# tensorlayer/HyperPose

Measured on NVIDIA H100. Metric: frames/sec end-to-end (conv+PAF parse) OpenPose-COCO 368x656, higher is better.
Workload: dtype f16 operands, f32 accumulate (conv); f32/f64 (parse)

## Files before the change

### hyperpose_b200/capi.py

```python
from __future__ import annotations

import ctypes as C
import os
import struct

import numpy as np

PKG = os.path.dirname(os.path.abspath(__file__))
LIB_PATH = os.path.join(PKG, "libhyperpose_b200.so")

N_PARTS, N_PAIRS = 18, 19
HP_OK, HP_ERR_ARG, HP_ERR_CAPACITY, HP_ERR_UNSUPPORTED, HP_ERR_CUDA, HP_ERR_BATCH = 0, -1, -2, -3, -4, -5

PART_DT = np.dtype({"names": ["has_value", "x", "y", "score"], "formats": ["<i4", "<f4", "<f4", "<f4"]})
HUMAN_DT = np.dtype([("parts", PART_DT, (N_PARTS,)), ("score", "<f4")])
PEAK_DT = np.dtype([("part_id", "<i4"), ("x", "<i4"), ("y", "<i4"), ("score", "<f4"), ("id", "<i4")])
CONN_DT = np.dtype([("cid1", "<i4"), ("cid2", "<i4"), ("score", "<f4")])
assert HUMAN_DT.itemsize == 292

EXPORTS = [
    "hp_last_error", "hp_device_count", "hp_version",
    "hp_paf_create", "hp_paf_destroy", "hp_paf_set_conf_thresh", "hp_paf_set_paf_thresh", "hp_paf_set_capacity",
    "hp_paf_process_host", "hp_paf_process_host_batched", "hp_paf_process_device", "hp_paf_fetch",
    "hp_paf_debug_peaks", "hp_paf_debug_connections", "hp_paf_launch_count", "hp_paf_copy_results_device", "hp_paf_debug_timing",
# ... 151 lines not shown
        _bind_engine(L)
        L._engine_bound = True
    check(L.hp_handoff_enable(1 if on else 0))


EXPORTS += [
    "hp_engine_create", "hp_engine_destroy", "hp_engine_info", "hp_engine_infer_u8_host", "hp_engine_infer_u8_device",
    "hp_engine_infer_f32_host", "hp_engine_outputs", "hp_engine_read_outputs_host", "hp_engine_copy_outputs_device", "hp_engine_sync",
    "hp_engine_launch_count", "hp_engine_debug_read_buffer", "hp_engine_debug_write_buffer", "hp_engine_debug_run_ops",
    "hp_pose_run_u8_host", "hp_engine_stage_frame_u8", "hp_engine_infer_staged", "hp_engine_debug_read_frames", "hp_engine_set_output_override", "hp_engine_set_profiling", "hp_engine_get_profile",
    "hp_engine_read_outputs_frames", "hp_engine_head_type", "hp_handoff_enable", "hp_handoff_stats",
    "hp_pose_submit_u8_host", "hp_pose_collect", "hp_pose_stats", "hp_paf_prepare", "hp_paf_state", "hp_paf_copy_results_host_async",
    "hp_paf_grow_capacity", "hp_pool_create", "hp_pool_destroy", "hp_pool_size", "hp_pool_set_capacity", "hp_pool_run_u8_host",
    "hp_pool_set_output_override", "hp_pool_launch_count", "hp_default_device", "hp_handoff_device_of",
    "hp_engine_create_ex", "hp_engine_dtype", "hp_pose_submit_u8_device", "hp_engine_debug_op_kernel",
    "hp_engine_debug_op_epilogue",
    "hp_engine_calibrate_u8", "hp_pack_int8_calibrated",
]


def _bind_engine(L):
    vp, ip = C.c_void_p, C.POINTER(C.c_int)
    L.hp_engine_create.argtypes = [C.POINTER(vp), vp, C.c_size_t, C.c_int, C.c_int, C.c_int, C.c_double, C.c_int, C.c_int]
    L.hp_engine_create_ex.argtypes = [C.POINTER(vp), vp, C.c_size_t, C.c_int, C.c_int, C.c_int, C.c_double, C.c_int, C.c_int, C.c_int]
    L.hp_engine_dtype.argtypes = [vp]
    L.hp_engine_destroy.argtypes = [vp]
    L.hp_engine_destroy.restype = None
    L.hp_engine_info.argtypes = [vp, ip, ip, ip, ip, ip, ip, ip, C.POINTER(C.c_double)]
    L.hp_engine_infer_u8_host.argtypes = [vp, vp, C.c_int]
    L.hp_engine_infer_u8_device.argtypes = [vp, vp, C.c_int, vp]
    L.hp_engine_infer_f32_host.argtypes = [vp, vp, C.c_int]
    L.hp_engine_outputs.argtypes = [vp, C.POINTER(vp), C.POINTER(vp), C.POINTER(vp)]
    L.hp_engine_read_outputs_host.argtypes = [vp, vp, vp, C.c_int]
    L.hp_engine_sync.argtypes = [vp]
    L.hp_engine_copy_outputs_device.argtypes = [vp, vp, vp, C.c_int, vp]
    L.hp_engine_launch_count.argtypes = [vp]
    L.hp_engine_launch_count.restype = C.c_longlong
    L.hp_engine_debug_read_buffer.argtypes = [vp, C.c_int, vp, C.c_int, ip, ip, ip]
    L.hp_engine_debug_write_buffer.argtypes = [vp, C.c_int, vp, C.c_int]
    L.hp_engine_debug_run_ops.argtypes = [vp, C.c_int, C.c_int, C.c_int]
    L.hp_engine_debug_op_kernel.argtypes = [vp, C.c_int, C.c_char_p, C.c_int]
    L.hp_engine_debug_op_epilogue.argtypes = [vp, C.c_int, ip]
    L.hp_engine_calibrate_u8.argtypes = [vp, vp, C.c_int, vp, C.c_int]
    L.hp_pack_int8_calibrated.argtypes = [vp, C.c_size_t]
    L.hp_pose_run_u8_host.argtypes = [vp, vp, vp, C.c_int, vp, C.c_int, ip]
    L.hp_engine_stage_frame_u8.argtypes = [vp, C.c_int, vp, C.c_int, C.c_int, C.c_int]
    L.hp_engine_infer_staged.argtypes = [vp, C.c_int]
    L.hp_engine_debug_read_frames.argtypes = [vp, vp, C.c_int]
    L.hp_engine_set_output_override.argtypes = [vp, vp, vp]
    L.hp_engine_set_profiling.argtypes = [vp, C.c_int]
    L.hp_engine_get_profile.argtypes = [vp, vp, vp, vp, C.c_int, ip, C.POINTER(C.c_longlong)]
    L.hp_engine_read_outputs_frames.argtypes = [vp, C.POINTER(vp), C.POINTER(vp), C.c_int, C.c_int]
    L.hp_engine_head_type.argtypes = [vp]
    L.hp_handoff_enable.argtypes = [C.c_int]
    L.hp_handoff_stats.argtypes = [C.POINTER(C.c_longlong)] * 4
    L.hp_pose_submit_u8_host.argtypes = [vp, vp, vp, C.c_int, ip]
    L.hp_pose_submit_u8_device.argtypes = [vp, vp, vp, C.c_int, ip]
# ... 143 lines not shown
        return out

    def debug_run_ops(self, first: int, last: int, n: int):
        check(lib().hp_engine_debug_run_ops(self._h, first, last, n))

    def debug_op_kernel(self, op: int) -> str:
        buf = C.create_string_buffer(64)
        check(lib().hp_engine_debug_op_kernel(self._h, op, buf, len(buf)))
        return buf.value.decode()

    def debug_op_epilogue(self, op: int) -> str:
        v = C.c_int(0)
        check(lib().hp_engine_debug_op_epilogue(self._h, op, C.byref(v)))
        return "tma" if v.value else "reg"

    def set_output_override(self, d_conf_ptr: int, d_paf_ptr: int):
        check(lib().hp_engine_set_output_override(self._h, d_conf_ptr, d_paf_ptr))

    def set_profiling(self, enable: bool):
        check(lib().hp_engine_set_profiling(self._h, 1 if enable else 0))

    def get_profile(self):
        cap = 1024
        ms = np.zeros(cap, np.float64); ty = np.zeros(cap, np.int32); fl = np.zeros(cap, np.float64)
        n, runs = C.c_int(), C.c_longlong()
        check(lib().hp_engine_get_profile(self._h, ms.ctypes.data, ty.ctypes.data, fl.ctypes.data, cap, C.byref(n), C.byref(runs)))
        return ms[:n.value], ty[:n.value], fl[:n.value], runs.value

    def run_pose(self, parser: "PafParser", frames: np.ndarray, cap: int = 128):
        frames = np.ascontiguousarray(frames, np.uint8)
# ... 242 lines not shown
```

### hyperpose_b200/csrc/conv_wgmma.cuh

```cuda
#pragma once
#include <cuda.h>
#include <cuda_fp16.h>
#include <cuda_runtime.h>
#include <stdint.h>

#include <type_traits>

namespace hpb {

constexpr int CONV_BLOCK_M = 128;
constexpr int CONV_BLOCK_K = 64;
constexpr int TF32_BLOCK_K = 32;
constexpr int CONV_MAX_STAGES = 8;
constexpr int CONV_THREADS = 384;
constexpr int CONV_A_BYTES = CONV_BLOCK_M * 128;
constexpr size_t CONV_SMEM_LIMIT = 227 * 1024;

enum ConvOutMode : int {
    OUT_F16_NHWC = 0,
    OUT_F32_NCHW_SPLIT = 1,
};

struct ConvParams {
    int Nb, H, W;
// ... 9 lines not shown
    int out_mode;
    void* out; void* out2;
    int out_ld, out_ch_off;
    int split;
    const void* res;
    int res_ld, res_ch_off;
    int res_mode;
    const float* post_w; const float* post_b; const float* post_a;
    const uint8_t* frames;
    int in_h, in_w, stem_stride, stem_pad_h, stem_pad_w, flip;
    double factor;
    float mean[3];
    const float* mul;
    float out_inv_scale, res_scale;
    int in_g_stride;
};

template <typename T> struct ConvAcc { using type = float; };
template <> struct ConvAcc<int8_t> { using type = int; };

namespace ptx {

__device__ __forceinline__ uint32_t smem_u32(const void* p) { return (uint32_t)__cvta_generic_to_shared(p); }

__device__ __forceinline__ void mbar_init(uint32_t bar, uint32_t count)
{
    asm volatile("mbarrier.init.shared::cta.b64 [%0], %1;" ::"r"(bar), "r"(count) : "memory");
}
__device__ __forceinline__ void mbar_expect_tx(uint32_t bar, uint32_t bytes)
{
// ... 51 lines not shown
        "cp.async.bulk.tensor.4d.shared::cluster.global.im2col.mbarrier::complete_tx::bytes [%0], [%1, {%3, %4, %5, %6}], [%2], {%7, %8};"
        ::"r"(dst), "l"(m), "r"(bar), "r"(c), "r"(w), "r"(h), "r"(n), "h"((unsigned short)offw), "h"((unsigned short)offh)
        : "memory");
}
__device__ __forceinline__ void tma_store_2d(const CUtensorMap* m, uint32_t src, int c0, int c1)
{
    asm volatile("cp.async.bulk.tensor.2d.global.shared::cta.bulk_group [%0, {%2, %3}], [%1];" ::"l"(m), "r"(src), "r"(c0), "r"(c1) : "memory");
}
__device__ __forceinline__ void tma_load_2d(uint32_t dst, const CUtensorMap* m, uint32_t bar, int c0, int c1)
{
    asm volatile(
        "cp.async.bulk.tensor.2d.shared::cluster.global.mbarrier::complete_tx::bytes [%0], [%1, {%3, %4}], [%2];"
        ::"r"(dst), "l"(m), "r"(bar), "r"(c0), "r"(c1)
        : "memory");
}
__device__ __forceinline__ void pdl_launch_dependents() { asm volatile("griddepcontrol.launch_dependents;" ::: "memory"); }
__device__ __forceinline__ void pdl_wait() { asm volatile("griddepcontrol.wait;" ::: "memory"); }
__device__ __forceinline__ float round_tf32(float x)
{
    uint32_t r;
    asm("cvt.rna.tf32.f32 %0, %1;" : "=r"(r) : "f"(x));
    return __uint_as_float(r);
}

__device__ __forceinline__ uint64_t make_sw128_kmajor_desc(uint32_t smem_addr)
{
    uint64_t d = 0;
    d |= (uint64_t)((smem_addr & 0x3ffffu) >> 4);
    d |= (uint64_t)1 << 16;
    d |= (uint64_t)(1024u >> 4) << 32;
// ... 265 lines not shown
                }
            }
        }
        vals[j] = __float2half_rn(v);
    }
    const uint4* v4 = (const uint4*)vals;
#pragma unroll
    for (int i = 0; i < 8; ++i) o[i ^ oswz] = v4[i];
}

__device__ __forceinline__ int8_t quantize_i8(float y, float inv_s)
{
    return (int8_t)min(max(__float2int_rn(__fmul_rn(y, inv_s)), -127), 127);
}

template <typename T, int BN, bool kRes, int kStemR = 0>
__global__ void __launch_bounds__(CONV_THREADS, 1)
conv_wgmma_kernel(const __grid_constant__ CUtensorMap tmap_a, const __grid_constant__ CUtensorMap tmap_b, const ConvParams p)
{
    constexpr bool kF16 = std::is_same<T, __half>::value;
    constexpr bool kI8 = std::is_same<T, int8_t>::value;
    constexpr int BK = 128 / (int)sizeof(T);
    constexpr int STAGE_BYTES = CONV_A_BYTES + BN * 128;
    extern __shared__ uint8_t smem_raw[];
    ptx::pdl_launch_dependents();
    uint8_t* smem = (uint8_t*)(((uintptr_t)smem_raw + 1023) & ~(uintptr_t)1023);
    uint64_t* full_bar = (uint64_t*)(smem + (size_t)p.num_stages * STAGE_BYTES);
    uint64_t* empty_bar = full_bar + CONV_MAX_STAGES;

    const int wg = threadIdx.x >> 7, warp = threadIdx.x >> 5, lane = threadIdx.x & 31;
    const int n_tiles_g = p.cout_g_pad / BN;
    const int total_tiles = p.m_tiles * p.groups * n_tiles_g;
    const int chunks = p.cin_g / BK;
    const int ksteps = p.R * p.S * chunks;

    if (threadIdx.x == 0) {
        ptx::prefetch_tmap(&tmap_a);
        ptx::prefetch_tmap(&tmap_b);
        for (int i = 0; i < p.num_stages; ++i) {
            ptx::mbar_init(ptx::smem_u32(full_bar + i), kStemR ? 129 : 1);
            ptx::mbar_init(ptx::smem_u32(empty_bar + i), 8);
        }
        ptx::fence_barrier_init();
    }
    __syncthreads();
    ptx::pdl_wait();

    if constexpr (kStemR > 0) {
        if (wg == 0) {
            const int row = threadIdx.x;
            const int total_px = p.Nb * p.H * p.W;
            int stage = 0;
            uint32_t phase = 0;
// ... 48 lines not shown
                            ptx::mbar_expect_tx(fb, (uint32_t)STAGE_BYTES);
                            ptx::tma_load_im2col_4d(ptx::smem_u32(sa), &tmap_a, fb, a_ch0 + c * BK, q0.w - pad_w, q0.h - pad_h, q0.n, s, r);
                            ptx::tma_load_2d(ptx::smem_u32(sa + CONV_A_BYTES), &tmap_b, fb, kcol, b_row);
                            ring.step(p.num_stages);
                        }
            }
        }
        return;
    }

    const int half = wg - 1;
    const int row0 = half * 64 + (warp & 3) * 16 + (lane >> 2);
    const int col0 = 2 * (lane & 3);
    const int total_px = p.Nb * p.H * p.W;
    const uint32_t smem0 = ptx::smem_u32(smem);
    typename ConvAcc<T>::type acc[BN / 2];
    RingPos ring;
    for (int tile = blockIdx.x; tile < total_tiles; tile += gridDim.x) {
        const ConvTile t = decode_tile(p, tile, n_tiles_g);
        int prev = 0;
        for (int ks = 0; ks < ksteps; ++ks) {
            const uint32_t sa = smem0 + (uint32_t)(ring.slot * STAGE_BYTES);
            const uint64_t da = ptx::make_sw128_kmajor_desc(sa + (uint32_t)(half * 64 * 128)), db = ptx::make_sw128_kmajor_desc(sa + CONV_A_BYTES);
            ptx::mbar_wait(ptx::smem_u32(full_bar + ring.slot), ring.phase);
            ptx::fence_acc(acc);
            ptx::wgmma_fence();
#pragma unroll
            for (int k = 0; k < 4; ++k)
                ptx::wgmma<T, BN>(acc, da + (uint64_t)(k * 2), db + (uint64_t)(k * 2), (ks | k) != 0 ? 1u : 0u);
            ptx::wgmma_commit();
            ptx::fence_acc(acc);
            if (ks > 0) {
                ptx::wgmma_wait<1>();
                if (lane == 0) ptx::mbar_arrive(ptx::smem_u32(empty_bar + prev));
            }
            prev = ring.slot;
            ring.step(p.num_stages);
        }
        ptx::wgmma_wait<0>();
        ptx::fence_acc(acc);
        if (lane == 0) ptx::mbar_arrive(ptx::smem_u32(empty_bar + prev));

        const float* bias = p.bias + t.g * p.cout_g_pad + t.n0;
        const float* alpha = p.alpha + t.g * p.cout_g_pad + t.n0;
        const int n_valid = min(BN, p.cout_g - t.n0);
        const int och = p.out_ch_off + t.g * p.cout_g + t.n0;
        const bool pair_ok = ((och | p.out_ld) & 1) == 0;
#pragma unroll
        for (int h = 0; h < 2; ++h) {
            const int px = t.p0 + row0 + 8 * h;
            if (px >= total_px) continue;
            const size_t pix = (size_t)px;
            const PixelPos q = unflatten(p, px);
#pragma unroll
            for (int j = 0; j < BN / 8; ++j) {
                const int c = 8 * j + col0;
                if (c >= n_valid) break;
// ... 72 lines not shown
                    for (int e = 0; e < 2; ++e) {
                        if (e == 1 && !two) break;
                        const int ch = t.n0 + c + e;
                        const float y = e ? a1 : a0;
                        if (ch < p.split) {
                            ((float*)p.out)[(((size_t)q.n * p.split + ch) * p.H + q.h) * p.W + q.w] = y;
                        } else {
                            const int c2 = ch - p.split, n2 = p.cout_g - p.split;
                            ((float*)p.out2)[(((size_t)q.n * n2 + c2) * p.H + q.h) * p.W + q.w] = y;
                        }
                    }
                }
            }
        }
    }
}

constexpr size_t CONV_SMEM_FIXED = 1024  + 2 * CONV_MAX_STAGES * 8;
inline size_t conv_smem_bytes(int BN, int stages) { return CONV_SMEM_FIXED + (size_t)stages * (CONV_A_BYTES + BN * 128); }
inline int conv_pick_stages(int BN)
{
    int s = CONV_MAX_STAGES;
    while (s > 2 && conv_smem_bytes(BN, s) > CONV_SMEM_LIMIT) --s;
    return s;
}

constexpr int HALO_TH = 16, HALO_TW = 8;

constexpr int HALO_WIDE_PRODUCER_REGS = 40, HALO_WIDE_CONSUMER_REGS = 232;


#ifdef HPB_HALO_PHASES
enum { HALO_PH_TOTAL, HALO_PH_A_WAIT, HALO_PH_B_WAIT, HALO_PH_MMA_WAIT, HALO_PH_EPILOGUE, HALO_PH_TURN_WAIT, HALO_PH_STAGE_WAIT, HALO_PH_COUNT };
__device__ unsigned long long g_halo_phases[HALO_PH_COUNT];
#define HALO_PH_MARK(t) const long long t = clock64()
#define HALO_TIMED(i, ...) do { const long long t0_ = clock64(); __VA_ARGS__; ph[i] += clock64() - t0_; } while (0)
#define HALO_PH_ADD(i, t) (ph[i] += clock64() - (t))
#define HALO_PH_PARAM , long long (&ph)[HALO_PH_COUNT]
// ... 37 lines not shown
}
inline int halo_stage_bytes(int BN, HaloItem it) { return halo_shape(it, BN).stage_slots * BN * 128; }

namespace ptx {
__device__ __forceinline__ uint64_t make_sw128_kmajor_desc_at(uint32_t smem_addr, uint32_t sbo)
{
    uint64_t d = 0;
    d |= (uint64_t)((smem_addr & 0x3ffffu) >> 4);
    d |= (uint64_t)1 << 16;
    d |= (uint64_t)((sbo >> 4) & 0x3fffu) << 32;
    d |= (uint64_t)1 << 62;
    return d;
}
template <uint32_t N> __device__ __forceinline__ void setmaxnreg_dec() { asm volatile("setmaxnreg.dec.sync.aligned.u32 %0;" ::"n"(N)); }
template <uint32_t N> __device__ __forceinline__ void setmaxnreg_inc() { asm volatile("setmaxnreg.inc.sync.aligned.u32 %0;" ::"n"(N)); }
__device__ __forceinline__ void stmatrix_x4(uint32_t addr, uint32_t r0, uint32_t r1, uint32_t r2, uint32_t r3)
{
    asm volatile("stmatrix.sync.aligned.m8n8.x4.shared.b16 [%0], {%1, %2, %3, %4};" ::"r"(addr), "r"(r0), "r"(r1), "r"(r2), "r"(r3) : "memory");
}
__device__ __forceinline__ void st_shared_u32(uint32_t addr, uint32_t v) { asm volatile("st.shared.b32 [%0], %1;" ::"r"(addr), "r"(v) : "memory"); }
__device__ __forceinline__ void named_barrier_sync(int id, int threads) { asm volatile("bar.sync %0, %1;" ::"r"(id), "r"(threads) : "memory"); }
__device__ __forceinline__ void tma_store_4d(const CUtensorMap* m, uint32_t src, int c0, int c1, int c2, int c3)
{
    asm volatile("cp.async.bulk.tensor.4d.global.shared::cta.bulk_group [%0, {%2, %3, %4, %5}], [%1];"
                 ::"l"(m), "r"(src), "r"(c0), "r"(c1), "r"(c2), "r"(c3) : "memory");
}
__device__ __forceinline__ void bulk_commit() { asm volatile("cp.async.bulk.commit_group;" ::: "memory"); }
template <int N> __device__ __forceinline__ void bulk_wait_read() { asm volatile("cp.async.bulk.wait_group.read %0;" ::"n"(N) : "memory"); }
template <int N> __device__ __forceinline__ void bulk_wait() { asm volatile("cp.async.bulk.wait_group %0;" ::"n"(N) : "memory"); }
__device__ __forceinline__ uint32_t half2_bits(__half2 h) { return *reinterpret_cast<uint32_t*>(&h); }
}

template <int BN, bool kPool, int kBlocks>
__device__ __forceinline__ void halo_epilogue(const float (&acc)[kBlocks][BN / 2], const HaloParams& p, int n, int y0, int x0, int g, int n0,
                                              int row_base, int warp, int lane)
{
    const int col0 = 2 * (lane & 3);
    const int tx = lane >> 2;
    const float* bias = p.bias + g * p.cout_g_pad + n0;
    const float* alpha = p.alpha + g * p.cout_g_pad + n0;
    const int och = p.out_ch_off + g * p.cout_g + n0;
    const bool pair_ok = ((och | p.out_ld) & 1) == 0;
    if constexpr (kPool) {
#pragma unroll
        for (int m = 0; m < kBlocks; ++m) {
// ... 398 lines not shown
```

### hyperpose_b200/csrc/engine.cu

```cuda
#include <cuda.h>
#include <cuda_fp16.h>
#include <cuda_runtime.h>
#include <math.h>
#include <stdint.h>
#include <stdlib.h>
#include <string.h>

#include <algorithm>
#include <memory>
#include <string>
#include <vector>

#include "../../include/hyperpose_b200.h"
#include "common.h"
#include "conv_wgmma.cuh"
#include "helpers_tf32_int8.cuh"
#include "handoff.h"
#include "pair_math.cuh"
#include "pack_format.h"

namespace {
using namespace hpb;


// ... 480 lines not shown

int make_tmap_act_box(CUtensorMap* m, const __half* base, int N, int H, int W, int C, int ld, int box_w, int box_h, CUtensorMapSwizzle swizzle)
{
    const auto enc = (PFN_encodeTiled)driver_entry_point("cuTensorMapEncodeTiled");
    if (!enc) { set_error("cuTensorMapEncodeTiled entry point not available"); return HP_ERR_CUDA; }
    cuuint64_t dims[4] = { (cuuint64_t)C, (cuuint64_t)W, (cuuint64_t)H, (cuuint64_t)N };
    cuuint64_t strides[3] = { (cuuint64_t)ld * 2, (cuuint64_t)W * ld * 2, (cuuint64_t)H * W * ld * 2 };
    cuuint32_t box[4] = { 64, (cuuint32_t)box_w, (cuuint32_t)box_h, 1 };
    cuuint32_t estr[4] = { 1, 1, 1, 1 };
    CUresult r = enc(m, CU_TENSOR_MAP_DATA_TYPE_FLOAT16, 4, (void*)base, dims, strides, box, estr, CU_TENSOR_MAP_INTERLEAVE_NONE,
                     swizzle, CU_TENSOR_MAP_L2_PROMOTION_L2_256B, CU_TENSOR_MAP_FLOAT_OOB_FILL_NONE);
    if (r != CUDA_SUCCESS) { set_error("cuTensorMapEncodeTiled(box) failed: %d (N=%d H=%d W=%d C=%d ld=%d box %dx%d)", (int)r, N, H, W, C, ld, box_w, box_h); return HP_ERR_CUDA; }
    return HP_OK;
}

int round_up(int a, int b) { return (a + b - 1) / b * b; }

int pick_bn(int cout_g)
{
    if (cout_g <= 16) return 16;
    if (cout_g <= 32) return 32;
    if (cout_g <= 48) return 48;
    if (cout_g <= 64) return 64;
    if (cout_g <= 96) return 96;
    if (cout_g <= 128) return 128;
    int best = 128;
    for (int bn : { 96, 64 })
        if (round_up(cout_g, bn) < round_up(cout_g, best)) best = bn;
    return best;
}
// ... 52 lines not shown

struct EngOp {
    Launch launch = Launch::None;
    PackOp po;
    ConvPlan plan;
    float* d_dw = nullptr;
    CUtensorMap tmap_dw;
    int dwt_wbo = 0, dwt_hb = 0, dwt_tiles_x = 0, dwt_tiles_y = 0, dwt_stages = 0;
    size_t dwt_smem = 0;
};

struct EngOptions {
    enum { HALO_AUTO, HALO_NONE, HALO_ALL } halo = HALO_AUTO;
    bool halo_wide = true;
    bool halo_tma_store = true;
    bool stem3 = true;
    bool pool_fuse = true;
    bool dw1_fuse = true;
    bool dw_pair = true;
    bool dw_tma = true;
    int pifpaf_reserve_sms = 0;
};

inline int same_pad_before(int in, int k, int stride)
{
    const int out = (in + stride - 1) / stride;
    const int total = std::max((out - 1) * stride + k - in, 0);
    return total / 2;
}

// ... 93 lines not shown
    HaloParams& h = op.plan.hp;
    const int BN = op.plan.prm.BN;
    h.tma_store = e->opt.halo_tma_store && halo_tma_store_ok(h, BN);
    h.stage_bytes = h.tma_store ? halo_stage_bytes(BN, item) : 0;
    h.num_stages = conv_halo_pick_stages(h.R, h.S, BN, item, h.tma_store);
    op.plan.smem = conv_halo_smem_bytes(h.R, h.S, BN, h.num_stages, item, h.tma_store);
    op.plan.halo_item = item;
    op.plan.halo_pool = pool;
    op.launch = Launch::Halo;
    if (!h.tma_store) return HP_OK;
    const int oh = pool ? h.H / 2 : h.H, ow = pool ? h.W / 2 : h.W, box = pool ? HALO_TW / 2 : HALO_TW;
    return make_tmap_act_box(&op.plan.tmap_o, h.out, e->max_batch, oh, ow, h.out_ch_off + h.groups * h.cout_g, h.out_ld, box, box,
                             CU_TENSOR_MAP_SWIZZLE_128B);
}

bool halo_wide_faster(int R, long wide_items, int sms)
{
    return R == 7 && wide_items >= sms;
}

bool halo_pp_exists(int R, int BN) { return R == 3 && (BN == 64 || BN == 128); }
bool halo_pp_faster(int chunks, bool pooled, long items, int sms) { return (chunks >= 4 || pooled) && items >= 2L * sms; }

HaloItem pick_halo_item(const hp_engine* e, const EngOp& op, bool pooled)
{
    const HaloParams& h = op.plan.hp;
    const int BN = op.plan.prm.BN, sms = e->num_sms - e->reserve_sms;
    const long tiles = (long)h.Nb * h.tiles_x * h.tiles_y, n_tiles = (long)h.groups * (h.cout_g_pad / BN);
    const bool all = e->opt.halo == EngOptions::HALO_ALL;
    if (!e->opt.halo_wide) return HaloItem::Narrow;
// ... 73 lines not shown
    }
    HP_CUDA_TRY(cudaMalloc(&pl.d_w, w.size() * es));
    HP_CUDA_TRY(cudaMalloc(&pl.d_bias, bias.size() * sizeof(float)));
    HP_CUDA_TRY(cudaMalloc(&pl.d_alpha, alpha.size() * sizeof(float)));
    HP_CUDA_TRY(cudaMemcpy(pl.d_w, tf32 ? (const void*)w.data() : i8 ? (const void*)wq.data() : (const void*)wh.data(), w.size() * es, cudaMemcpyHostToDevice));
    HP_CUDA_TRY(cudaMemcpy(pl.d_bias, bias.data(), bias.size() * sizeof(float), cudaMemcpyHostToDevice));
    HP_CUDA_TRY(cudaMemcpy(pl.d_alpha, alpha.data(), alpha.size() * sizeof(float), cudaMemcpyHostToDevice));

    ConvParams& p = pl.prm;
    memset(&p, 0, sizeof(p));
    p.Nb = e->max_batch; p.H = ib.H; p.W = ib.W;
    p.R = eR; p.S = eS; p.groups = G; p.cin_g = ecin;
    p.cout_g = cout_g; p.cout_g_pad = cout_pad; p.BN = BN;
    p.m_tiles = (int)(((size_t)e->max_batch * p.H * p.W + CONV_BLOCK_M - 1) / CONV_BLOCK_M);
    p.in_ch_off = (int)po.in_ch_off;
    p.num_stages = conv_pick_stages(BN);
    p.bias = pl.d_bias; p.alpha = pl.d_alpha;
    p.out_mode = (int)po.out_mode;
    if (po.out_mode == OUT_F32_NCHW_SPLIT) {
        p.out = e->d_conf; p.out2 = e->d_paf; p.split = (int)po.split;
        if ((int)po.split != (int)e->hdr.conf_channels || cout_g - (int)po.split != (int)e->hdr.paf_channels || G != 1) {
            set_error("engine: output conv must produce conf(%u)+paf(%u) channels", e->hdr.conf_channels, e->hdr.paf_channels);
            return HP_ERR_ARG;
        }
        if (e->hdr.head_type != 0 || ib.H != e->out_h || ib.W != e->out_w) {
            set_error("engine: output conv op %d reads a %dx%d buffer but the outputs are %dx%d conf/paf planes (head_type %u)",
                      (int)(&op - e->ops.data()), ib.H, ib.W, e->out_h, e->out_w, e->hdr.head_type);
            return HP_ERR_ARG;
        }
    } else {
        const EngBuffer& ob = e->bufs[po.out_buf];
// ... 1 lines not shown
        p.out = ob.d; p.out_ld = ob.channels; p.out_ch_off = (int)po.out_ch_off;
        if (i8) p.out_inv_scale = 1.0f / e->act_scale[po.out_buf];
    }
    if (i8) { p.mul = pl.d_mul; p.in_g_stride = cin_g; }
    if (po.res_mode) {
        if (po.out_mode != OUT_F16_NHWC || po.res_buf >= e->bufs.size()) { set_error("engine: bad residual"); return HP_ERR_ARG; }
        const EngBuffer& rb = e->bufs[po.res_buf];
        if (rb.H != ib.H || rb.W != ib.W || (int)po.res_ch_off + G * cout_g > rb.channels || po.res_ch_off % 8 || cout_g % 16) { set_error("engine: residual buffer mismatch"); return HP_ERR_ARG; }
        p.res = rb.d; p.res_ld = rb.channels; p.res_ch_off = (int)po.res_ch_off; p.res_mode = (int)po.res_mode;
        if (i8) p.res_scale = e->act_scale[po.res_buf];
    }
    int rc = make_tmap_act_im2col(&pl.tmap_a, ib.d, e->max_batch, ib.H, ib.W, ib.channels, eR, eS, e->dtype);
    if (rc) return rc;
    rc = make_tmap_wgt(&pl.tmap_b, pl.d_w, G * cout_pad, K, BN, e->dtype);
    if (rc) return rc;
    pl.smem = conv_smem_bytes(BN, p.num_stages);
    pl.flops_per_frame = 2.0 * ib.H * ib.W * (double)G * cout_g * cin_g * R * S;
    op.launch = Launch::Conv;
    if (e->dtype != HP_DTYPE_F16) return HP_OK;
    pl.monotone_act = true;
    for (float a : alpha) if (!(a >= 0.f)) { pl.monotone_act = false; break; }
    const int ty = (ib.H + HALO_TH - 1) / HALO_TH, tx = (ib.W + HALO_TW - 1) / HALO_TW;
    const double waste = (double)ty * HALO_TH * tx * HALO_TW / ((double)ib.H * ib.W) - 1.0;
    const bool shape_ok = !im2col && eR == eS && (eR == 3 || eR == 5 || eR == 7) && !po.res_mode && po.out_mode == OUT_F16_NHWC;
    const bool rounds = (long)p.m_tiles * G * (cout_pad / BN) > e->num_sms - e->reserve_sms;
    const bool faster = (eR == 3 && waste <= 0.06) || (rounds && ecin >= 2 * CONV_BLOCK_K && waste <= 0.25);
    const bool want = e->opt.halo == EngOptions::HALO_AUTO ? faster : e->opt.halo == EngOptions::HALO_ALL;
    if (shape_ok && want) {
        const EngBuffer& ob = e->bufs[po.out_buf];
        HaloParams& h = pl.hp;
        memset(&h, 0, sizeof(h));
// ... 100 lines not shown
        HaloParams h = pl.hp;
        h.Nb = N;
        const int tiles = halo_shape(pl.halo_item, p.BN).tiles;
        const long items = ((long)N * h.tiles_x * h.tiles_y + tiles - 1) / tiles * h.groups * (h.cout_g_pad / p.BN);
        cudaLaunchAttribute at[1];
        const cudaLaunchConfig_t cfg = pdl_config((int)std::min<long>(e->num_sms - e->reserve_sms, items), CONV_THREADS, pl.smem, st, at);
        void* args[] = { (void*)&pl.tmap_x, (void*)&pl.tmap_b, (void*)&pl.tmap_o, (void*)&h };
        HP_CUDA_TRY(cudaLaunchKernelExC(&cfg, halo_kernel(p.BN, pl.halo_item, pl.halo_pool), args));
        return HP_OK;
    }
    p.m_tiles = (int)(((size_t)N * p.H * p.W + CONV_BLOCK_M - 1) / CONV_BLOCK_M);
    const int n_tiles = p.m_tiles * p.groups * (p.cout_g_pad / p.BN);
    const int grid = std::min(e->num_sms - e->reserve_sms, n_tiles);
    cudaLaunchAttribute at[1];
    const cudaLaunchConfig_t cfg = pdl_config(grid, CONV_THREADS, pl.smem, st, at);
    void* args[] = { (void*)&pl.tmap_a, (void*)&pl.tmap_b, (void*)&p };
    HP_CUDA_TRY(cudaLaunchKernelExC(&cfg, conv_kernel(e->dtype, p.res_mode != 0, p.BN, stem_R), args));
    return HP_OK;
}

bool collect_one(hp_engine* e, bool blocking)
{
    if (e->ev_tail >= e->ev_head) return false;
    const size_t n = e->ops.size();
    cudaEvent_t* set = e->ev.data() + (size_t)(e->ev_tail % hp_engine::EV_DEPTH) * (n + 1);
    if (!blocking && cudaEventQuery(set[n]) != cudaSuccess) { cudaGetLastError(); return false; }
    cudaEventSynchronize(set[n]);
    for (size_t i = 0; i < n; ++i) {
        float ms = 0.f;
        if (cudaEventElapsedTime(&ms, set[i], set[i + 1]) == cudaSuccess) e->op_ms_sum[i] += ms;
    }
// ... 321 lines not shown
        }
    }
    HP_CUDA_TRY(cudaSetDevice(device));
    cudaDeviceProp prop;
    HP_CUDA_TRY(cudaGetDeviceProperties(&prop, device));
    if (prop.major != 9) { set_error("hp_engine_create: device is sm_%d%d; this engine is wgmma/TMA code for sm_90a only", prop.major, prop.minor); return HP_ERR_UNSUPPORTED; }

    hp_engine* e = new hp_engine();
    e->device = device; e->dtype = dtype; e->in_h = in_h; e->in_w = in_w; e->max_batch = max_batch;
    e->factor = factor; e->flip_rgb = flip_rgb; e->hdr = hdr; e->num_sms = prop.multiProcessorCount;
    e->act_scale = std::move(act_scale);
    EngOptions& opt = e->opt;
    if (const char* v = getenv("HPB_HALO")) opt.halo = strcmp(v, "all") == 0 ? EngOptions::HALO_ALL : EngOptions::HALO_NONE;
    opt.halo_wide = !getenv("HPB_HALO_NARROW");
    opt.halo_tma_store = !getenv("HPB_HALO_REG_EPILOGUE");
    opt.stem3 = !getenv("HPB_NO_STEM3");
    opt.pool_fuse = !getenv("HPB_NO_POOL_FUSE");
    opt.dw1_fuse = !getenv("HPB_NO_DW1_FUSE");
    opt.dw_pair = !getenv("HPB_NO_DW_DUAL");
    opt.dw_tma = !getenv("HPB_NO_DW_TMA");
    const char* rs = getenv("HPB_PIFPAF_RESERVE_SMS");
    opt.pifpaf_reserve_sms = std::max(0, std::min(rs ? atoi(rs) : std::min(max_batch, 16), e->num_sms / 2));
    const uint8_t* ptr = (const uint8_t*)pack + sizeof(PackHeader);
    const PackBuffer* pb = (const PackBuffer*)ptr;
    const PackOp* pops = (const PackOp*)(ptr + hdr.n_buffers * sizeof(PackBuffer));
    std::vector<float> blob(hdr.blob_floats);
    memcpy(blob.data(), (const uint8_t*)pops + hdr.n_ops * sizeof(PackOp), hdr.blob_floats * sizeof(float));

    int rc = HP_OK;
    auto fail = [&](int code) { free_engine(e); return code; };
// ... 163 lines not shown
            const PackOp& q = e->ops[k].po;
            if (reads_buffer(q, c.po.out_buf)) safe = false;
            else if (q.type != OP_IM2COL3 && q.type != OP_PIFPAF_HEAD && q.type != OP_PPN_HEAD && q.out_mode != OUT_F32_NCHW_SPLIT && q.out_buf == c.po.out_buf) {
                const int qc = q.type == OP_CONV ? (int)q.groups * (int)q.cout_g : (int)q.cout_g;
                if (q.out_ch_off <= c.po.out_ch_off && (int)q.out_ch_off + qc >= (int)c.po.out_ch_off + Ctot) rewritten = true; else safe = false;
            }
        }
        if (!safe) continue;
        const EngBuffer& ob = e->bufs[d.po.out_buf];
        if ((int)d.po.out_ch_off + Ctot > ob.channels) continue;
        c.plan.prm.out = ob.d; c.plan.prm.out_ld = ob.channels; c.plan.prm.out_ch_off = (int)d.po.out_ch_off;
        c.plan.prm.post_w = d.d_dw; c.plan.prm.post_b = d.d_dw + Ctot; c.plan.prm.post_a = d.d_dw + 2 * (size_t)Ctot;
        d.launch = Launch::None;
        if (!rewritten) e->bufs[c.po.out_buf].fused_away = true;
    }
    size_t dwt_max = 0;
    for (EngOp& a : e->ops) {
        const PackOp& po = a.po;
        if (!opt.dw_tma || a.launch != Launch::DwCol || po.cout_g % 64 || po.in_buf == po.out_buf) continue;
        const EngBuffer& ib = e->bufs[po.in_buf];
        const int C = (int)po.cout_g, halo = 2 * dw_dilation(po);
        const int nx = (ib.W + 63 - halo) / (64 - halo), wbo = (ib.W + nx - 1) / nx, bw = wbo + halo;
        int hb = 2;
        for (int cand : { 8, 6, 4, 3, 2 }) {
            if (cand > std::max(2, ib.H) || (size_t)(cand + halo) * bw * 128 > (size_t)DWT_STAGE_MAX) continue;
            const size_t items = (size_t)e->max_batch * ((ib.H + cand - 1) / cand) * nx * (C / 64);
            hb = cand;
            if (items >= 2 * (size_t)e->num_sms) break;
        }
        const size_t stage = (size_t)(hb + halo) * bw * 128;
// ... 389 lines not shown
        s = s.back() == '>' ? s.substr(0, s.size() - 1) + "," + d + ">" : s + "<" + d + ">";
    }
    if ((int)s.size() >= cap) { set_error("hp_engine_debug_op_kernel: %zu-character name, capacity %d", s.size(), cap); return HP_ERR_CAPACITY; }
    memcpy(name, s.c_str(), s.size() + 1);
    return HP_OK;
}

int hp_engine_debug_op_epilogue(const hp_engine* e, int op, int* tma_store)
{
    if (!e || op < 0 || op >= (int)e->ops.size() || !tma_store) { set_error("hp_engine_debug_op_epilogue: bad argument"); return HP_ERR_ARG; }
    const EngOp& o = e->ops[op];
    *tma_store = o.launch == Launch::Halo && o.plan.hp.tma_store ? 1 : 0;
    return HP_OK;
}

long long hp_engine_launch_count(const hp_engine* e) { return e ? e->launches : 0; }

int hp_engine_set_output_override(hp_engine* e, const float* d_conf, const float* d_paf)
{
    if (!e) return HP_ERR_ARG;
    e->override_conf = d_conf;
    e->override_paf = d_paf;
    return HP_OK;
}

int hp_engine_set_profiling(hp_engine* e, int enable)
{
    if (!e) return HP_ERR_ARG;
    HP_CUDA_TRY(cudaSetDevice(e->device));
    if (enable && e->ev.empty()) {
// ... 326 lines not shown
```

### include/hyperpose_b200.h

```cpp
#ifndef HYPERPOSE_B200_H
#define HYPERPOSE_B200_H

#include <stddef.h>
#include <stdint.h>

#ifdef __cplusplus
extern "C" {
#endif

#define HP_N_PARTS 18
#define HP_N_PAIRS 19

typedef enum hp_status {
    HP_OK = 0,
    HP_ERR_ARG = -1,
    HP_ERR_CAPACITY = -2,
    HP_ERR_UNSUPPORTED = -3,
    HP_ERR_CUDA = -4,
    HP_ERR_BATCH = -5
} hp_status;

typedef struct hp_body_part {
    int32_t has_value;
    float x, y, score;
// ... 90 lines not shown
int hp_engine_infer_f32_host(hp_engine* e, const float* nchw, int N);
int hp_engine_outputs(hp_engine* e, const float** d_conf, const float** d_paf, void** stream);
int hp_engine_read_outputs_host(hp_engine* e, float* conf, float* paf, int N);
int hp_engine_read_outputs_frames(hp_engine* e, float* const* conf_frames, float* const* paf_frames, int N, int publish);
int hp_engine_head_type(const hp_engine* e);
int hp_handoff_enable(int on);
int hp_handoff_stats(long long* published, long long* hits, long long* batch_parses, long long* misses);
int hp_engine_copy_outputs_device(hp_engine* e, float* d_conf, float* d_paf, int N, void* stream);
int hp_engine_sync(hp_engine* e);
long long hp_engine_launch_count(const hp_engine* e);
int hp_engine_debug_read_buffer(hp_engine* e, int buf, void* out_f16, int N, int* H, int* W, int* C);
int hp_engine_debug_write_buffer(hp_engine* e, int buf, const void* in_f16, int N);
int hp_engine_debug_run_ops(hp_engine* e, int first_op, int last_op, int N);
int hp_engine_debug_op_kernel(const hp_engine* e, int op, char* name, int cap);
int hp_engine_debug_op_epilogue(const hp_engine* e, int op, int* tma_store);

int hp_engine_set_output_override(hp_engine* e, const float* d_conf, const float* d_paf);
int hp_engine_set_profiling(hp_engine* e, int enable);
int hp_engine_get_profile(hp_engine* e, double* ms_per_op, int* op_type, double* flops_per_op, int cap, int* n_ops, long long* runs);

int hp_pose_run_u8_host(hp_engine* e, hp_paf* parser, const uint8_t* frames, int N, hp_human* out, int cap, int* n_out);
int hp_pose_submit_u8_host(hp_engine* e, hp_paf* parser, const uint8_t* frames, int N, int* ticket);
int hp_pose_submit_u8_device(hp_engine* e, hp_paf* parser, const uint8_t* d_frames, int N, int* ticket);
int hp_pose_collect(hp_engine* e, int ticket, hp_human* out, int cap, int* n_out);
int hp_pose_stats(const hp_engine* e, long long* graph_captures, long long* graph_launches);
int hp_pose_submit_pifpaf_u8_host(hp_engine* e, hp_pifpaf* decoder, const uint8_t* frames, int N, int* ticket);
int hp_pose_submit_pifpaf_u8_device(hp_engine* e, hp_pifpaf* decoder, const uint8_t* d_frames, int N, int* ticket);
int hp_pifpaf_pipeline_info(hp_pifpaf* p, void** stream, void** inputs_free_event, int* hcap);
int hp_pifpaf_copy_results_host_async(hp_pifpaf* p, hp_human* pin_humans, int* pin_counts_flags, int N, void* stream);
int hp_pifpaf_grow_capacity(hp_pifpaf* p, int flags);
// ... 22 lines not shown
```

Baseline: 1007.

## Add TMA-store epilogue for f16 NHWC conv kernels via stmatrix staging

Adds an alternative epilogue for the wgmma conv kernel that writes activated f16 outputs into a swizzled shared-memory staging buffer with stmatrix and then issues TMA 2D bulk stores, replacing per-thread scattered global stores. It is enabled by default for f16 NHWC outputs with BN 64/128 and suitable alignment, and falls back to the register epilogue for partial tiles. The staging buffer takes extra shared memory, which can reduce the number of pipeline stages chosen. The epilogue also adds named-barrier syncs and bulk-group waits.

Measured after the change: 1100, median of 6. 1.09x the previous value.

```diff
diff --git a/hyperpose_b200/capi.py b/hyperpose_b200/capi.py
--- a/hyperpose_b200/capi.py
+++ b/hyperpose_b200/capi.py
@@ -189,7 +189,7 @@
     "hp_paf_grow_capacity", "hp_pool_create", "hp_pool_destroy", "hp_pool_size", "hp_pool_set_capacity", "hp_pool_run_u8_host",
     "hp_pool_set_output_override", "hp_pool_launch_count", "hp_default_device", "hp_handoff_device_of",
     "hp_engine_create_ex", "hp_engine_dtype", "hp_pose_submit_u8_device", "hp_engine_debug_op_kernel",
-    "hp_engine_debug_op_epilogue",
+    "hp_engine_debug_op_epilogue", "hp_engine_debug_op_conv_epilogue",
     "hp_engine_calibrate_u8", "hp_pack_int8_calibrated",
 ]
 
@@ -216,6 +216,7 @@
     L.hp_engine_debug_run_ops.argtypes = [vp, C.c_int, C.c_int, C.c_int]
     L.hp_engine_debug_op_kernel.argtypes = [vp, C.c_int, C.c_char_p, C.c_int]
     L.hp_engine_debug_op_epilogue.argtypes = [vp, C.c_int, ip]
+    L.hp_engine_debug_op_conv_epilogue.argtypes = [vp, C.c_int, ip]
     L.hp_engine_calibrate_u8.argtypes = [vp, vp, C.c_int, vp, C.c_int]
     L.hp_pack_int8_calibrated.argtypes = [vp, C.c_size_t]
     L.hp_pose_run_u8_host.argtypes = [vp, vp, vp, C.c_int, vp, C.c_int, ip]
@@ -389,6 +390,11 @@
         check(lib().hp_engine_debug_op_epilogue(self._h, op, C.byref(v)))
         return "tma" if v.value else "reg"
 
+    def debug_op_conv_epilogue(self, op: int) -> str:
+        v = C.c_int(0)
+        check(lib().hp_engine_debug_op_conv_epilogue(self._h, op, C.byref(v)))
+        return "tma" if v.value else "reg"
+
     def set_output_override(self, d_conf_ptr: int, d_paf_ptr: int):
         check(lib().hp_engine_set_output_override(self._h, d_conf_ptr, d_paf_ptr))
 
diff --git a/hyperpose_b200/csrc/conv_wgmma.cuh b/hyperpose_b200/csrc/conv_wgmma.cuh
--- a/hyperpose_b200/csrc/conv_wgmma.cuh
+++ b/hyperpose_b200/csrc/conv_wgmma.cuh
@@ -47,6 +47,7 @@
     const float* mul;
     float out_inv_scale, res_scale;
     int in_g_stride;
+    int tma_store;
 };
 
 template <typename T> struct ConvAcc { using type = float; };
@@ -128,6 +129,15 @@
         ::"r"(dst), "l"(m), "r"(bar), "r"(c0), "r"(c1)
         : "memory");
 }
+__device__ __forceinline__ void stmatrix_x4(uint32_t addr, uint32_t r0, uint32_t r1, uint32_t r2, uint32_t r3)
+{
+    asm volatile("stmatrix.sync.aligned.m8n8.x4.shared.b16 [%0], {%1, %2, %3, %4};" ::"r"(addr), "r"(r0), "r"(r1), "r"(r2), "r"(r3) : "memory");
+}
+__device__ __forceinline__ void named_barrier_sync(int id, int threads) { asm volatile("bar.sync %0, %1;" ::"r"(id), "r"(threads) : "memory"); }
+__device__ __forceinline__ void bulk_commit() { asm volatile("cp.async.bulk.commit_group;" ::: "memory"); }
+template <int N> __device__ __forceinline__ void bulk_wait_read() { asm volatile("cp.async.bulk.wait_group.read %0;" ::"n"(N) : "memory"); }
+template <int N> __device__ __forceinline__ void bulk_wait() { asm volatile("cp.async.bulk.wait_group %0;" ::"n"(N) : "memory"); }
+__device__ __forceinline__ uint32_t half2_bits(__half2 h) { return *reinterpret_cast<uint32_t*>(&h); }
 __device__ __forceinline__ void pdl_launch_dependents() { asm volatile("griddepcontrol.launch_dependents;" ::: "memory"); }
 __device__ __forceinline__ void pdl_wait() { asm volatile("griddepcontrol.wait;" ::: "memory"); }
 __device__ __forceinline__ float round_tf32(float x)
@@ -423,18 +433,84 @@
     return (int8_t)min(max(__float2int_rn(__fmul_rn(y, inv_s)), -127), 127);
 }
 
+template <int BN, bool kRes>
+__device__ __forceinline__ void conv_epilogue_tma(const float (&acc)[BN / 2], const ConvParams& p, const ConvTile& t, const CUtensorMap* tmap_o,
+                                                  uint32_t slot, int half, int warp, int lane)
+{
+    static_assert(BN == 64 || BN == 128, "one TMA box per 64-channel slice, at most two");
+    constexpr int kSliceBytes = 64 * 128;
+    const bool leader = (threadIdx.x & 127) == 0;
+    const int bar_id = 1 + half;
+    const int col0 = 2 * (lane & 3);
+    const float* bias = p.bias + t.g * p.cout_g_pad + t.n0;
+    const float* alpha = p.alpha + t.g * p.cout_g_pad + t.n0;
+    const int n_valid = min(BN, p.cout_g - t.n0);
+    const int och = p.out_ch_off + t.g * p.cout_g + t.n0;
+    const int px0 = t.p0 + half * 64;
+    if (leader) ptx::bulk_wait_read<0>();
+    ptx::named_barrier_sync(bar_id, 128);
+    const int r = lane & 7, i = lane >> 3;
+#pragma unroll
+    for (int jb = 0; jb < BN / 32; ++jb) {
+#pragma unroll
+        for (int h = 0; h < 2; ++h) {
+            const size_t pix = (size_t)(px0 + (warp & 3) * 16 + 8 * h + (lane >> 2));
+            uint32_t v[4];
+#pragma unroll
+            for (int k = 0; k < 4; ++k) {
+                const int j = 4 * jb + k, c = 8 * j + col0;
+                const bool real = c < n_valid;
+                float a0 = acc[4 * j + 2 * h] + __ldg(bias + c), a1 = acc[4 * j + 2 * h + 1] + __ldg(bias + c + 1);
+                float r0 = 0.f, r1 = 0.f;
+                if (kRes && p.res_mode && real) {
+                    const size_t ri = pix * p.res_ld + p.res_ch_off + t.g * p.cout_g + t.n0 + c;
+                    const float2 rf = __half22float2(*((const __half2*)p.res + ri / 2)); r0 = rf.x; r1 = rf.y;
+                }
+                if (kRes && p.res_mode == 1) { a0 += r0; a1 += r1; }
+                a0 = a0 > 0.f ? a0 : a0 * __ldg(alpha + c);
+                a1 = a1 > 0.f ? a1 : a1 * __ldg(alpha + c + 1);
+                if (kRes && p.res_mode == 2) { a0 += r0; a1 += r1; }
+                __half2 h2 = __floats2half2_rn(a0, a1);
+                if (p.post_w && real) {
+                    const int pc = t.g * p.cout_g + t.n0 + c;
+                    const float2 x = __half22float2(h2);
+                    float y0 = fmaf(x.x, __ldg(p.post_w + pc), 0.f) + __ldg(p.post_b + pc);
+                    float y1 = fmaf(x.y, __ldg(p.post_w + pc + 1), 0.f) + __ldg(p.post_b + pc + 1);
+                    y0 = y0 > 0.f ? y0 : y0 * __ldg(p.post_a + pc);
+                    y1 = y1 > 0.f ? y1 : y1 * __ldg(p.post_a + pc + 1);
+                    h2 = __floats2half2_rn(y0, y1);
+                }
+                v[k] = ptx::half2_bits(h2);
+            }
+            const int j = 4 * jb + i, row = (warp & 3) * 16 + 8 * h + r;
+            ptx::stmatrix_x4(slot + (uint32_t)((j >> 3) * kSliceBytes + row * 128 + (((j & 7) ^ r) << 4)), v[0], v[1], v[2], v[3]);
+        }
+    }
+    ptx::fence_proxy_async();
+    ptx::named_barrier_sync(bar_id, 128);
+    if (leader) {
+        ptx::tma_store_2d(tmap_o, slot, och, px0);
+        if (BN == 128 && t.n0 + 64 < p.cout_g)
+            ptx::tma_store_2d(tmap_o, slot + (uint32_t)kSliceBytes, och + 64, px0);
+        ptx::bulk_commit();
+    }
+}
+
 template <typename T, int BN, bool kRes, int kStemR = 0>
 __global__ void __launch_bounds__(CONV_THREADS, 1)
-conv_wgmma_kernel(const __grid_constant__ CUtensorMap tmap_a, const __grid_constant__ CUtensorMap tmap_b, const ConvParams p)
+conv_wgmma_kernel(const __grid_constant__ CUtensorMap tmap_a, const __grid_constant__ CUtensorMap tmap_b, const __grid_constant__ CUtensorMap tmap_o,
+                  const ConvParams p)
 {
     constexpr bool kF16 = std::is_same<T, __half>::value;
     constexpr bool kI8 = std::is_same<T, int8_t>::value;
     constexpr int BK = 128 / (int)sizeof(T);
     constexpr int STAGE_BYTES = CONV_A_BYTES + BN * 128;
+    constexpr bool kTmaForm = kF16 && (BN == 64 || BN == 128);
     extern __shared__ uint8_t smem_raw[];
     ptx::pdl_launch_dependents();
     uint8_t* smem = (uint8_t*)(((uintptr_t)smem_raw + 1023) & ~(uintptr_t)1023);
-    uint64_t* full_bar = (uint64_t*)(smem + (size_t)p.num_stages * STAGE_BYTES);
+    uint8_t* s_stage = smem + (size_t)p.num_stages * STAGE_BYTES;
+    uint64_t* full_bar = (uint64_t*)(s_stage + (p.tma_store ? 2 * BN * 128 : 0));
     uint64_t* empty_bar = full_bar + CONV_MAX_STAGES;
 
     const int wg = threadIdx.x >> 7, warp = threadIdx.x >> 5, lane = threadIdx.x & 31;
@@ -446,6 +522,7 @@
     if (threadIdx.x == 0) {
         ptx::prefetch_tmap(&tmap_a);
         ptx::prefetch_tmap(&tmap_b);
+        if (kTmaForm && p.tma_store) ptx::prefetch_tmap(&tmap_o);
         for (int i = 0; i < p.num_stages; ++i) {
             ptx::mbar_init(ptx::smem_u32(full_bar + i), kStemR ? 129 : 1);
             ptx::mbar_init(ptx::smem_u32(empty_bar + i), 8);
@@ -524,6 +601,7 @@
     const int col0 = 2 * (lane & 3);
     const int total_px = p.Nb * p.H * p.W;
     const uint32_t smem0 = ptx::smem_u32(smem);
+    const bool tma = kTmaForm && p.tma_store;
     typename ConvAcc<T>::type acc[BN / 2];
     RingPos ring;
     for (int tile = blockIdx.x; tile < total_tiles; tile += gridDim.x) {
@@ -551,6 +629,12 @@
         ptx::fence_acc(acc);
         if (lane == 0) ptx::mbar_arrive(ptx::smem_u32(empty_bar + prev));
 
+        if constexpr (kTmaForm) {
+            if (tma && t.p0 + half * 64 + 64 <= total_px) {
+                conv_epilogue_tma<BN, kRes>(acc, p, t, &tmap_o, ptx::smem_u32(s_stage + (size_t)half * BN * 128), half, warp, lane);
+                continue;
+            }
+        }
         const float* bias = p.bias + t.g * p.cout_g_pad + t.n0;
         const float* alpha = p.alpha + t.g * p.cout_g_pad + t.n0;
         const int n_valid = min(BN, p.cout_g - t.n0);
@@ -653,14 +737,18 @@
             }
         }
     }
+    if (tma && (threadIdx.x & 127) == 0) ptx::bulk_wait<0>();
 }
 
 constexpr size_t CONV_SMEM_FIXED = 1024  + 2 * CONV_MAX_STAGES * 8;
-inline size_t conv_smem_bytes(int BN, int stages) { return CONV_SMEM_FIXED + (size_t)stages * (CONV_A_BYTES + BN * 128); }
-inline int conv_pick_stages(int BN)
+inline size_t conv_smem_bytes(int BN, int stages, bool tma_store)
+{
+    return CONV_SMEM_FIXED + (size_t)stages * (CONV_A_BYTES + BN * 128) + (tma_store ? 2 * (size_t)BN * 128 : 0);
+}
+inline int conv_pick_stages(int BN, bool tma_store)
 {
     int s = CONV_MAX_STAGES;
-    while (s > 2 && conv_smem_bytes(BN, s) > CONV_SMEM_LIMIT) --s;
+    while (s > 2 && conv_smem_bytes(BN, s, tma_store) > CONV_SMEM_LIMIT) --s;
     return s;
 }
 
@@ -728,21 +816,12 @@
 }
 template <uint32_t N> __device__ __forceinline__ void setmaxnreg_dec() { asm volatile("setmaxnreg.dec.sync.aligned.u32 %0;" ::"n"(N)); }
 template <uint32_t N> __device__ __forceinline__ void setmaxnreg_inc() { asm volatile("setmaxnreg.inc.sync.aligned.u32 %0;" ::"n"(N)); }
-__device__ __forceinline__ void stmatrix_x4(uint32_t addr, uint32_t r0, uint32_t r1, uint32_t r2, uint32_t r3)
-{
-    asm volatile("stmatrix.sync.aligned.m8n8.x4.shared.b16 [%0], {%1, %2, %3, %4};" ::"r"(addr), "r"(r0), "r"(r1), "r"(r2), "r"(r3) : "memory");
-}
 __device__ __forceinline__ void st_shared_u32(uint32_t addr, uint32_t v) { asm volatile("st.shared.b32 [%0], %1;" ::"r"(addr), "r"(v) : "memory"); }
-__device__ __forceinline__ void named_barrier_sync(int id, int threads) { asm volatile("bar.sync %0, %1;" ::"r"(id), "r"(threads) : "memory"); }
 __device__ __forceinline__ void tma_store_4d(const CUtensorMap* m, uint32_t src, int c0, int c1, int c2, int c3)
 {
     asm volatile("cp.async.bulk.tensor.4d.global.shared::cta.bulk_group [%0, {%2, %3, %4, %5}], [%1];"
                  ::"l"(m), "r"(src), "r"(c0), "r"(c1), "r"(c2), "r"(c3) : "memory");
 }
-__device__ __forceinline__ void bulk_commit() { asm volatile("cp.async.bulk.commit_group;" ::: "memory"); }
-template <int N> __device__ __forceinline__ void bulk_wait_read() { asm volatile("cp.async.bulk.wait_group.read %0;" ::"n"(N) : "memory"); }
-template <int N> __device__ __forceinline__ void bulk_wait() { asm volatile("cp.async.bulk.wait_group %0;" ::"n"(N) : "memory"); }
-__device__ __forceinline__ uint32_t half2_bits(__half2 h) { return *reinterpret_cast<uint32_t*>(&h); }
 }
 
 template <int BN, bool kPool, int kBlocks>
diff --git a/hyperpose_b200/csrc/engine.cu b/hyperpose_b200/csrc/engine.cu
--- a/hyperpose_b200/csrc/engine.cu
+++ b/hyperpose_b200/csrc/engine.cu
@@ -518,6 +518,20 @@
     return HP_OK;
 }
 
+int make_tmap_pixel_rows(CUtensorMap* m, const __half* base, long pixels, int C, int ld)
+{
+    const auto enc = (PFN_encodeTiled)driver_entry_point("cuTensorMapEncodeTiled");
+    if (!enc) { set_error("cuTensorMapEncodeTiled entry point not available"); return HP_ERR_CUDA; }
+    cuuint64_t dims[2] = { (cuuint64_t)C, (cuuint64_t)pixels };
+    cuuint64_t strides[1] = { (cuuint64_t)ld * 2 };
+    cuuint32_t box[2] = { 64, 64 };
+    cuuint32_t estr[2] = { 1, 1 };
+    CUresult r = enc(m, CU_TENSOR_MAP_DATA_TYPE_FLOAT16, 2, (void*)base, dims, strides, box, estr, CU_TENSOR_MAP_INTERLEAVE_NONE,
+                     CU_TENSOR_MAP_SWIZZLE_128B, CU_TENSOR_MAP_L2_PROMOTION_L2_256B, CU_TENSOR_MAP_FLOAT_OOB_FILL_NONE);
+    if (r != CUDA_SUCCESS) { set_error("cuTensorMapEncodeTiled(pixel rows) failed: %d (pixels=%ld C=%d ld=%d)", (int)r, pixels, C, ld); return HP_ERR_CUDA; }
+    return HP_OK;
+}
+
 int round_up(int a, int b) { return (a + b - 1) / b * b; }
 
 int pick_bn(int cout_g)
@@ -600,6 +614,7 @@
     enum { HALO_AUTO, HALO_NONE, HALO_ALL } halo = HALO_AUTO;
     bool halo_wide = true;
     bool halo_tma_store = true;
+    bool conv_tma_store = true;
     bool stem3 = true;
     bool pool_fuse = true;
     bool dw1_fuse = true;
@@ -723,6 +738,17 @@
                              CU_TENSOR_MAP_SWIZZLE_128B);
 }
 
+int set_conv_tma_store(const hp_engine* e, EngOp& op)
+{
+    ConvParams& p = op.plan.prm;
+    p.tma_store = e->opt.conv_tma_store && e->dtype == HP_DTYPE_F16 && p.out_mode == OUT_F16_NHWC && (p.BN == 64 || p.BN == 128) &&
+                  p.out_ld % 8 == 0 && p.out_ch_off % 8 == 0 && (p.groups * p.cout_g) % 8 == 0 && (p.groups == 1 || p.cout_g % p.BN == 0);
+    p.num_stages = conv_pick_stages(p.BN, p.tma_store);
+    op.plan.smem = conv_smem_bytes(p.BN, p.num_stages, p.tma_store);
+    if (!p.tma_store) return HP_OK;
+    return make_tmap_pixel_rows(&op.plan.tmap_o, (const __half*)p.out, (long)e->max_batch * p.H * p.W, p.out_ch_off + p.groups * p.cout_g, p.out_ld);
+}
+
 bool halo_wide_faster(int R, long wide_items, int sms)
 {
     return R == 7 && wide_items >= sms;
@@ -826,7 +852,7 @@
     p.cout_g = cout_g; p.cout_g_pad = cout_pad; p.BN = BN;
     p.m_tiles = (int)(((size_t)e->max_batch * p.H * p.W + CONV_BLOCK_M - 1) / CONV_BLOCK_M);
     p.in_ch_off = (int)po.in_ch_off;
-    p.num_stages = conv_pick_stages(BN);
+    p.num_stages = conv_pick_stages(BN, false);
     p.bias = pl.d_bias; p.alpha = pl.d_alpha;
     p.out_mode = (int)po.out_mode;
     if (po.out_mode == OUT_F32_NCHW_SPLIT) {
@@ -858,7 +884,7 @@
     if (rc) return rc;
     rc = make_tmap_wgt(&pl.tmap_b, pl.d_w, G * cout_pad, K, BN, e->dtype);
     if (rc) return rc;
-    pl.smem = conv_smem_bytes(BN, p.num_stages);
+    pl.smem = conv_smem_bytes(BN, p.num_stages, false);
     pl.flops_per_frame = 2.0 * ib.H * ib.W * (double)G * cout_g * cin_g * R * S;
     op.launch = Launch::Conv;
     if (e->dtype != HP_DTYPE_F16) return HP_OK;
@@ -989,7 +1015,7 @@
     const int grid = std::min(e->num_sms - e->reserve_sms, n_tiles);
     cudaLaunchAttribute at[1];
     const cudaLaunchConfig_t cfg = pdl_config(grid, CONV_THREADS, pl.smem, st, at);
-    void* args[] = { (void*)&pl.tmap_a, (void*)&pl.tmap_b, (void*)&p };
+    void* args[] = { (void*)&pl.tmap_a, (void*)&pl.tmap_b, (void*)&pl.tmap_o, (void*)&p };
     HP_CUDA_TRY(cudaLaunchKernelExC(&cfg, conv_kernel(e->dtype, p.res_mode != 0, p.BN, stem_R), args));
     return HP_OK;
 }
@@ -1341,6 +1367,7 @@
     if (const char* v = getenv("HPB_HALO")) opt.halo = strcmp(v, "all") == 0 ? EngOptions::HALO_ALL : EngOptions::HALO_NONE;
     opt.halo_wide = !getenv("HPB_HALO_NARROW");
     opt.halo_tma_store = !getenv("HPB_HALO_REG_EPILOGUE");
+    opt.conv_tma_store = !getenv("HPB_CONV_REG_EPILOGUE");
     opt.stem3 = !getenv("HPB_NO_STEM3");
     opt.pool_fuse = !getenv("HPB_NO_POOL_FUSE");
     opt.dw1_fuse = !getenv("HPB_NO_DW1_FUSE");
@@ -1534,6 +1561,11 @@
         d.launch = Launch::None;
         if (!rewritten) e->bufs[c.po.out_buf].fused_away = true;
     }
+    for (EngOp& c : e->ops) {
+        if (c.launch != Launch::Conv && c.launch != Launch::ConvStem) continue;
+        if (int rc = set_conv_tma_store(e, c)) return fail(rc);
+        max_smem = std::max(max_smem, c.plan.smem);
+    }
     size_t dwt_max = 0;
     for (EngOp& a : e->ops) {
         const PackOp& po = a.po;
@@ -1953,6 +1985,14 @@
     return HP_OK;
 }
 
+int hp_engine_debug_op_conv_epilogue(const hp_engine* e, int op, int* tma_store)
+{
+    if (!e || op < 0 || op >= (int)e->ops.size() || !tma_store) { set_error("hp_engine_debug_op_conv_epilogue: bad argument"); return HP_ERR_ARG; }
+    const EngOp& o = e->ops[op];
+    *tma_store = (o.launch == Launch::Conv || o.launch == Launch::ConvStem) && o.plan.prm.tma_store ? 1 : 0;
+    return HP_OK;
+}
+
 long long hp_engine_launch_count(const hp_engine* e) { return e ? e->launches : 0; }
 
 int hp_engine_set_output_override(hp_engine* e, const float* d_conf, const float* d_paf)
diff --git a/include/hyperpose_b200.h b/include/hyperpose_b200.h
--- a/include/hyperpose_b200.h
+++ b/include/hyperpose_b200.h
@@ -128,6 +128,7 @@
 int hp_engine_debug_run_ops(hp_engine* e, int first_op, int last_op, int N);
 int hp_engine_debug_op_kernel(const hp_engine* e, int op, char* name, int cap);
 int hp_engine_debug_op_epilogue(const hp_engine* e, int op, int* tma_store);
+int hp_engine_debug_op_conv_epilogue(const hp_engine* e, int op, int* tma_store);
 
 int hp_engine_set_output_override(hp_engine* e, const float* d_conf, const float* d_paf);
 int hp_engine_set_profiling(hp_engine* e, int enable);
```
